# garymm/starflate

Measured on AMD Instinct MI355X. Metric: compress MiB/s + ratio vs zlib -6, 1 GiB synthetic; 1/2/4/8 GPU, higher is better.
Workload: dtype u8

## Files before the change

### starflate_amd/csrc/sf_capi.hip

```cpp
#include "../../include/starflate_hip.h"
#include "sf_device.h"

#include <dlfcn.h>
#include <stdio.h>
#include <stdlib.h>
#include <string.h>
#include <algorithm>
#include <memory>
#include <new>
#include <thread>
#include <vector>

struct sfh_ctx {
  int device = 0;
  hipStream_t stream = nullptr;
  sf::Workspace ws{};
  uint32_t cap_chunks = 0;
  uint32_t cap_batch = 0;
  uint32_t cap_dtok = 0;
  size_t seginfo_cap = 0;
  size_t sums_cap = 0;
  uint32_t last_chunks = 0;
  uint32_t last_block_bytes = 0;
  bool index_valid = false;
// ... 261 lines not shown
    SF_HIP(hipEventSynchronize(ctx->ev_batch[b % sfh_ctx::kPipe]), "wait for a batch");
    const size_t end = (size_t)ctx->h_tot[b % sfh_ctx::kPipe];
    if (end > pipe->cap) { pipe->overflow = true; return SFH_OK; }
    if (end > pipe->copied)
      SF_HIP(hipMemcpyAsync(pipe->dst + pipe->copied, (const uint8_t*)d_dst + pipe->copied, end - pipe->copied,
                            hipMemcpyDeviceToHost, ctx->s_out), "D2H");
    pipe->copied = end;
    return SFH_OK;
  };
  uint32_t bi = 0;
  for (uint32_t c0 = 0; c0 < nchunks; c0 += batch, ++bi) {
    const uint32_t nb = std::min(batch, nchunks - c0);
    const bool first = c0 == 0, last = c0 + nb == nchunks;
    const uint8_t* bsrc = (const uint8_t*)d_src + (size_t)c0 * sf::kChunk;
    const size_t bn = std::min((size_t)nb * sf::kChunk, n - (size_t)c0 * sf::kChunk);
    if (pipe && bn) {
      SF_HIP(hipMemcpyAsync(const_cast<uint8_t*>(bsrc), pipe->src + (size_t)c0 * sf::kChunk, bn, hipMemcpyHostToDevice, ctx->s_in), "H2D");
      SF_HIP(hipEventRecord(ctx->ev_in[bi % sfh_ctx::kPipe], ctx->s_in), "event");
      SF_HIP(hipStreamWaitEvent(s, ctx->ev_in[bi % sfh_ctx::kPipe], 0), "wait for the input");
    }
    sf::Workspace w = ctx->ws;
    w.offsets += c0;
    w.subidx += (size_t)c0 * 2 * sf::kSubRegions;
    sf::Options bo = ko;
    bo.final_stream = last ? ko.final_stream : 0u;
    hipEvent_t* ev = prof ? &ctx->ev[(size_t)bi * sfh_ctx::kEvPerBatch] : nullptr;
    if (ev) SF_HIP(hipEventRecord(ev[0], s), "event");
    SF_HIP(sf::launch_lz77(bsrc, bn, nb, w, bo, s), "launch k_lz77");
    if (ev) SF_HIP(hipEventRecord(ev[1], s), "event");
    SF_HIP(sf::launch_plan(bn, nb, w, bo, s), "launch k_plan");
    if (ev) SF_HIP(hipEventRecord(ev[2], s), "event");
    SF_HIP(sf::launch_scan(nb, w, sf::wrapper_header_bytes(o.container), !first, d_out_n, s), "launch k_scan");
    if (ev) SF_HIP(hipEventRecord(ev[3], s), "event");
    SF_HIP(sf::launch_emit(bsrc, bn, nb, w, (uint8_t*)d_dst, s), "launch k_emit");
    if (ev) SF_HIP(hipEventRecord(ev[4], s), "event");
    if (pipe) {
      if (bi >= 1 && (rc = drain(bi - 1)) != SFH_OK) return rc;
      SF_HIP(hipMemcpyAsync(&ctx->h_tot[bi % sfh_ctx::kPipe], d_out_n, sizeof(uint64_t), hipMemcpyDeviceToHost, s), "copy size");
      SF_HIP(hipEventRecord(ctx->ev_batch[bi % sfh_ctx::kPipe], s), "event");
    }
  }
  if (pipe && (rc = drain(bi - 1)) != SFH_OK) return rc;
  if (o.container) {
    SF_HIP(sf::launch_checksum((const uint8_t*)d_src, n, nchunks, o.container, ctx->ws.sums, s), "launch k_checksum");
    SF_HIP(sf::launch_wrap(ctx->ws.sums, nchunks, n, o.container, (uint8_t*)d_dst, d_out_n, nullptr, s), "launch k_wrap");
  }
  if (prof) {
    SF_HIP(hipEventRecord(ctx->ev[(size_t)nbatches * sfh_ctx::kEvPerBatch], s), "event");
    ctx->ev_batches = nbatches;
  }
  ctx->ev_valid = prof;
  ctx->index_valid = true;
  return mark_call_end(ctx, s);
}

int stage_tables(sfh_ctx* ctx, size_t bytes) {
  if (!ctx->ev_tab) SF_HIP(hipEventCreateWithFlags(&ctx->ev_tab, hipEventDisableTiming), "event");
  if (ctx->tab_pending) SF_HIP(hipEventSynchronize(ctx->ev_tab), "wait for the previous call's table copy");
  ctx->tab_pending = false;
  if (ctx->h_tab_cap < bytes) {
    if (ctx->h_tab) (void)hipHostFree(ctx->h_tab);
    ctx->h_tab = nullptr;
    ctx->h_tab_cap = 0;
    const hipError_t e = hipHostMalloc((void**)&ctx->h_tab, bytes, hipHostMallocDefault);
    if (e != hipSuccess) return fail(ctx, SFH_E_NOMEM, "pinned descriptor tables", e);
    ctx->h_tab_cap = bytes;
  }
// ... 123 lines not shown

  ctx->index_valid = false;
  ctx->last_chunks = lbs.back().nchunks;
  const bool prof = ctx->profiling != 0;
  if ((rc = order_behind_last_call(ctx, s)) != SFH_OK) return rc;
  SF_HIP(hipMemcpyAsync(ctx->d_tab, ctx->h_tab, bytes, hipMemcpyHostToDevice, s), "descriptor tables");
  SF_HIP(hipEventRecord(ctx->ev_tab, s), "event");
  ctx->tab_pending = true;
  const uint32_t nbatches = (uint32_t)lbs.size();
  ctx->ev_valid = false;
  if (prof) {
    const size_t need = (size_t)nbatches * sfh_ctx::kEvPerBatch + 1;
    while (ctx->ev.size() < need) {
      hipEvent_t e = nullptr;
      SF_HIP(hipEventCreate(&e), "event");
      ctx->ev.push_back(e);
    }
  }
  const uint64_t hdr = sf::wrapper_header_bytes(o.container);
  for (uint32_t bi = 0; bi < nbatches; ++bi) {
    const LaunchBatch& b = lbs[bi];
    const sf::BatchTables bt{d_strips + b.s0, b.nstrips, d_chunks + b.c0, d_items + b.i0, b.nitems};
    sf::Workspace w = ctx->ws;
    w.offsets += b.c0;
    w.subidx += (size_t)b.c0 * 2 * sf::kSubRegions;
    hipEvent_t* ev = prof ? &ctx->ev[(size_t)bi * sfh_ctx::kEvPerBatch] : nullptr;
    if (ev) SF_HIP(hipEventRecord(ev[0], s), "event");
    SF_HIP(sf::launch_lz77(nullptr, 0, b.nchunks, ctx->ws, ko, s, &bt), "launch k_lz77");
    if (ev) SF_HIP(hipEventRecord(ev[1], s), "event");
    SF_HIP(sf::launch_plan(0, b.nchunks, ctx->ws, ko, s, &bt), "launch k_plan");
    if (ev) SF_HIP(hipEventRecord(ev[2], s), "event");
    SF_HIP(sf::launch_scan(b.nchunks, w, hdr, false, d_out_n, s, &bt), "launch k_scan");
    if (ev) SF_HIP(hipEventRecord(ev[3], s), "event");
    SF_HIP(sf::launch_emit(nullptr, 0, b.nchunks, w, nullptr, s, &bt), "launch k_emit");
    if (ev) SF_HIP(hipEventRecord(ev[4], s), "event");
  }
  SF_HIP(sf::launch_batch_index(d_chunks, d_ixrows, d_items, ctx->ws.offsets, d_out_n, nchunks, ctx->d_bix, s), "launch k_batch_index");
  if (o.container) {
    SF_HIP(sf::launch_checksum_batch(d_chunks, nchunks, o.container, ctx->ws.sums, s), "launch k_checksum");
    SF_HIP(sf::launch_wrap_batch(ctx->ws.sums, d_wraps, (uint32_t)count, o.container, d_out_n, s), "launch k_wrap");
  }
  if (prof) {
    SF_HIP(hipEventRecord(ctx->ev[(size_t)nbatches * sfh_ctx::kEvPerBatch], s), "event");
    ctx->ev_batches = nbatches;
  }
  ctx->ev_valid = prof;
  ctx->bix_valid = true;
  ctx->bix_items = count;
  ctx->bix_entries = (size_t)nchunks + count;
  return mark_call_end(ctx, s);
}

int check_inflate_batch(sfh_ctx* ctx, size_t count, const void* const* srcs, const uint64_t* src_n, const uint64_t* index,
                        const uint32_t* subindex, void* const* dsts, const uint64_t* dst_n, const uint32_t* block_bytes,
                        uint32_t container, const uint32_t* status, bool dev) {
  if (!ctx || container > SFH_GZIP) return fail(ctx, SFH_E_INVALID_ARG, "argument (container)", hipSuccess);
  if (count == 0) return SFH_OK;
  if (!srcs || !src_n || !dsts || !dst_n || !status) return fail(ctx, SFH_E_INVALID_ARG, "null array", hipSuccess);
  if (count > ((size_t)1 << 31) - 1) return fail(ctx, SFH_E_INVALID_ARG, "too many items", hipSuccess);
  if (subindex && !index) return fail(ctx, SFH_E_INVALID_ARG, "a sub-index without an index", hipSuccess);
  if (dev && (((uintptr_t)index & 7) || ((uintptr_t)subindex & 3) || ((uintptr_t)status & 3)))
    return fail(ctx, SFH_E_INVALID_ARG, "device pointer alignment (index 8, sub-index 4, status 4)", hipSuccess);
  uint64_t segs = 0;
  for (size_t i = 0; i < count; ++i) {
    if ((!srcs[i] && src_n[i]) || (!dsts[i] && dst_n[i])) return fail(ctx, SFH_E_INVALID_ARG, "null item pointer", hipSuccess);
    if (dev && (((uintptr_t)srcs[i] & 3) || ((uintptr_t)dsts[i] & 15)))
      return fail(ctx, SFH_E_INVALID_ARG, "device pointer alignment (src 4, dst 16)", hipSuccess);
// ... 1005 lines not shown
```

### starflate_amd/csrc/sf_device.h

```cpp
#pragma once
#include <hip/hip_runtime.h>
#include <stdint.h>

namespace sf {

constexpr uint32_t kChunk = 32768;
constexpr uint32_t kWindow = 32768;
constexpr uint32_t kStep = 1024;
constexpr uint32_t kHashBits = 13;
constexpr uint32_t kMaxStrip = 1u << 24;
constexpr uint32_t kRegion = 512;
constexpr uint32_t kSubBytes = 1024;
constexpr uint32_t kCap = 16;
constexpr uint32_t kMinMatch = 4;
constexpr uint32_t kFar4 = 4096;
constexpr uint32_t kSkipSlack = 128;
constexpr uint32_t kSkipProbe = 2048;
constexpr uint32_t kItemsSkipped = 0x80000000u;
constexpr uint32_t kSubRegions = kChunk / kSubBytes;
constexpr uint32_t kTokMatch = 0x80000000u;
constexpr uint32_t kTokRegion = 0x40000000u;
constexpr uint32_t kItemTok = 0x8000u;
constexpr uint32_t kItemRegion = 0x4000u;
constexpr uint32_t kItemRegionShift = 9;
// ... 148 lines not shown
  uint32_t hist;
};
constexpr uint32_t kSegWrapped = 0x80000000u;
struct InflateStrip {
  uint32_t seg0, nseg;
};
struct InflateItem {
  const uint8_t* src;
  uint64_t src_n;
  uint64_t dst_n;
  uint64_t* implied;
  const uint64_t* ix0;
  uint32_t seg0, nseg;
  uint32_t wst;
  uint32_t want;
  uint32_t isize;
  uint32_t pad;
};
static_assert(sizeof(InflateSeg) == 48 && sizeof(InflateStrip) == 8 && sizeof(InflateItem) == 64, "decoder descriptor rows");
struct BatchTables {
  const BatchStrip* strips;
  uint32_t nstrips;
  const BatchChunk* chunks;
  BatchItem* items;
  uint32_t nitems;
};

hipError_t launch_lz77(const uint8_t* src, uint64_t n, uint32_t nchunks, const Workspace& ws,
                       const Options& opt, hipStream_t s, const BatchTables* bt = nullptr);
hipError_t launch_plan(uint64_t n, uint32_t nchunks, const Workspace& ws, const Options& opt,
                       hipStream_t s, const BatchTables* bt = nullptr);
hipError_t launch_scan(uint32_t nchunks, const Workspace& ws, uint64_t base, bool carry, uint64_t* d_total, hipStream_t s,
                       const BatchTables* bt = nullptr);
hipError_t launch_emit(const uint8_t* src, uint64_t n, uint32_t nchunks, const Workspace& ws,
                       uint8_t* dst, hipStream_t s, const BatchTables* bt = nullptr);
hipError_t launch_batch_index(const BatchChunk* chunks, const BatchIndexRow* rows, const BatchItem* pieces, const uint64_t* offsets,
                              const uint64_t* total, uint32_t nchunks, uint64_t* index, hipStream_t s);
hipError_t init_kernels();

uint32_t wrapper_header_bytes(uint32_t kind);
hipError_t launch_checksum(const uint8_t* src, uint64_t n, uint32_t nchunks, uint32_t kind, uint32_t* sums,
                           hipStream_t s);
hipError_t launch_wrap(const uint32_t* sums, uint32_t nchunks, uint64_t n, uint32_t kind, uint8_t* dst,
                       uint64_t* d_total, uint32_t* d_value, hipStream_t s);
hipError_t launch_checksum_batch(const BatchChunk* chunks, uint32_t nchunks, uint32_t kind, uint32_t* sums, hipStream_t s);
hipError_t launch_wrap_batch(const uint32_t* sums, const WrapItem* items, uint32_t nitems, uint32_t kind,
                             uint64_t* d_total, hipStream_t s);
hipError_t init_inflate_kernels();
hipError_t launch_inflate_tokens(const uint8_t* src, uint64_t src_n, const uint64_t* index, uint32_t nseg, uint64_t dst_n,
                                 uint32_t* tokens, SegInfo* info, uint32_t sps, bool speculate, hipStream_t s);
hipError_t launch_inflate_tokens_sub(const uint8_t* src, uint64_t src_n, const uint64_t* index, const uint32_t* subidx,
                                     uint32_t nseg, uint64_t dst_n, uint32_t* tokens, SegInfo* info, uint32_t sps,
                                     hipStream_t s);
hipError_t launch_inflate_bytes(const uint8_t* src, uint64_t src_n, uint32_t nseg, const uint32_t* tokens, SegInfo* info,
                                uint8_t* dst, uint32_t sps, hipStream_t s);
hipError_t launch_inflate_status(const SegInfo* info, uint32_t nseg, uint32_t* d_result, hipStream_t s);
hipError_t launch_inflate_tokens_batch(const InflateSeg* rows, uint32_t nseg, uint32_t* tokens, SegInfo* info, bool sub,
                                       bool speculate, hipStream_t s);
hipError_t launch_inflate_bytes_batch(const InflateSeg* rows, const InflateStrip* strips, uint32_t nstrips,
                                      const uint32_t* tokens, SegInfo* info, hipStream_t s);
hipError_t launch_inflate_head(InflateItem* items, uint32_t nitems, uint32_t container, InflateSeg* segs, BatchChunk* sums,
                               hipStream_t s);
hipError_t launch_inflate_fold(const InflateItem* items, uint32_t nitems, const SegInfo* info, const uint32_t* sums,
                               uint32_t container, uint32_t* status, hipStream_t s);

hipError_t run_lds_order_check(int op, uint32_t blocks, uint32_t iters, uint32_t* d_result, hipStream_t s);

// ... 5 lines not shown
```

### starflate_amd/csrc/sf_kernels.hip

```cpp
#include "sf_device.h"

#include <stdlib.h>

namespace sf {

__device__ __forceinline__ uint32_t len_symbol(uint32_t l3, uint32_t& ebits, uint32_t& eval) {
  if (l3 == 255) { ebits = 0; eval = 0; return 285; }
  if (l3 < 8) { ebits = 0; eval = 0; return 257 + l3; }
  const uint32_t e = (31 - __builtin_clz(l3)) - 2;
  ebits = e;
  eval = l3 & ((1u << e) - 1);
  return 257 + 4 * e + 4 + ((l3 >> e) & 3);
}
__device__ __forceinline__ uint32_t dist_symbol(uint32_t d1, uint32_t& ebits, uint32_t& eval) {
  if (d1 < 4) { ebits = 0; eval = 0; return d1; }
  const uint32_t hb = 31 - __builtin_clz(d1);
  const uint32_t e = hb - 1;
  ebits = e;
  eval = d1 & ((1u << e) - 1);
  return 2 * hb + ((d1 >> e) & 1);
}
__device__ __forceinline__ uint32_t dist_symbol_of(uint32_t d1) {
  const uint32_t x = d1 > 2u ? d1 : 2u;
  const uint32_t hb = 31 - __builtin_clz(x);
// ... 1314 lines not shown
      } else {
        q = (r - 1) / 6u;
        rem = (r - 1) - 6u * q;
        cnt = 1 + q + ((rem >= 3) ? 1u : rem);
      }
    }
    const uint32_t incl = wave_incl_add(cnt);
    uint32_t k = base + total + incl - cnt;
    auto put = [&](uint32_t sym, uint32_t ext) {
      S.rle_sym[k] = (uint8_t)sym;
      S.rle_ext[k] = (uint8_t)ext;
      atomicAdd(&S.clfreq[sym], 1u);
      ++k;
    };
    if (start) {
      if (v == 0) {
        for (uint32_t c = 0; c < q; ++c) put(18, 138 - 11);
        if (rem >= 11) put(18, rem - 11);
        else if (rem >= 3) put(17, rem - 3);
        else for (uint32_t c = 0; c < rem; ++c) put(0, 0);
      } else {
        put(v, 0);
        for (uint32_t c = 0; c < q; ++c) put(16, 6 - 3);
        if (rem >= 3) put(16, rem - 3);
        else for (uint32_t c = 0; c < rem; ++c) put(v, 0);
      }
    }
    total += (uint32_t)__builtin_amdgcn_readlane((int)incl, 63);
  }
  return total;
}

__constant__ uint8_t c_cl_order[19] = {16, 17, 18, 0, 8, 7, 9, 6, 10, 5, 11, 4, 12, 3, 13, 2, 14, 1, 15};

template <int MODE>
__device__ __forceinline__ void plan_chunk(uint64_t n_total, uint32_t nchunks,
                                           uint32_t* __restrict__ hist, const uint32_t* __restrict__ ntok,
                                           ChunkPlan* __restrict__ plan, ChunkCodes* __restrict__ codes,
                                           uint32_t strategy, uint32_t final_stream,
                                           uint64_t* __restrict__ stamps, PlanTree* __restrict__ ptree,
                                           const BatchChunk* __restrict__ bchunks) {
  __shared__ PlanSmem S;
  uint32_t* const s_header = S.key + kHeaderAt;
  uint64_t st_t = stamps ? __builtin_amdgcn_s_memtime() : 0;
  uint32_t st_k = 0;
  auto stamp = [&]() {
    if (stamps) {
      const uint64_t now = __builtin_amdgcn_s_memtime();
      if (threadIdx.x == 0 && st_k < 8) stamps[((uint64_t)nchunks + blockIdx.x) * 8 + st_k] = now - st_t;
      st_t = now;
      ++st_k;
    }
  };
  const uint32_t lane = threadIdx.x;
  const uint32_t chunk = blockIdx.x;
  uint32_t n_raw;
  bool fin;
  if (bchunks) {
    const BatchChunk B = bchunks[chunk];
    n_raw = B.n_raw;
    fin = (B.item & 1u) && final_stream;
  } else {
    const uint64_t cbase = (uint64_t)chunk * kChunk;
    n_raw = (uint32_t)((n_total - cbase) < (uint64_t)kChunk ? (n_total - cbase) : kChunk);
    fin = (chunk + 1 == nchunks) && final_stream;
  }

  PlanTree* const T = ptree + chunk;
  if constexpr (MODE == 2) {
    if (T->done) return;
  }
  if (MODE == 1 && strategy == 0 && n_raw != 0 && ntok[chunk] == 0) {
    ChunkCodes& C0 = codes[chunk];
    for (uint32_t s0 = lane; s0 < 320; s0 += 64) C0.lens[s0] = 0;
    if (lane == 0) {
      C0.header[0] = fin ? 1u : 0u;
      ChunkPlan P;
      P.btype = 0;
      P.out_bytes = n_raw + 5;
      P.header_bits = 3;
      P.body_bits = 0;
      plan[chunk] = P;
      T->done = 1;
    }
    return;
  }
  uint32_t rawf[4] = {0, 0, 0, 0};
  if constexpr (MODE == 1) {
#pragma unroll
    for (uint32_t q = 0; q < 4; ++q) rawf[q] = hist[(uint64_t)chunk * kHistStride + kHistLen + lane + 64 * q];
  }
  for (uint32_t s = lane; s < 320; s += 64) S.freq[s] = hist[(uint64_t)chunk * kHistStride + s];
  for (uint32_t s = lane; s < 320; s += 64) S.lens[s] = 0;
  __syncthreads();
  if constexpr (MODE == 1) {
#pragma unroll
    for (uint32_t q = 0; q < 4; ++q) {
      uint32_t eb, ev;
      if (rawf[q]) atomicAdd(&S.freq[len_symbol(lane + 64 * q, eb, ev)], rawf[q]);
    }
    __syncthreads();
    if (lane < 29) hist[(uint64_t)chunk * kHistStride + 257 + lane] = S.freq[257 + lane];
  }

  stamp();
  if (MODE == 1 && strategy == 0) {
    uint32_t fixb = 0, extra = 0, tot = 0;
    for (uint32_t s0 = lane; s0 < 286; s0 += 64) tot += S.freq[s0];
    tot = wave_sum(tot);
    const uint32_t ltot = est_log2(tot);
    uint32_t ent = 0;
    for (uint32_t s0 = lane; s0 < 286; s0 += 64) {
      const uint32_t f = S.freq[s0];
      if (f) ent += f * (ltot - est_log2(f));
      fixb += f * fixed_ll_len(s0);
      if (s0 >= 257) extra += f * len_extra_of_sym(s0 - 257);
    }
    const uint32_t g = lane < 30 ? S.freq[kHistD + lane] : 0u;
    const uint32_t nmat = wave_sum(g);
    if (g) ent += g * (est_log2(nmat) - est_log2(g));
    if (lane < 30) extra += g * dist_extra_of_sym(lane);
    const uint32_t extra_all = wave_sum(extra);
    const uint32_t est_bits = (wave_sum(ent) >> 8) + extra_all + kEstHeaderBits;
    const uint32_t fixbits = 3 + wave_sum(fixb) + extra_all + 5 * nmat;
    const uint32_t est_b = fin ? (est_bits + 7) / 8 : (est_bits + 3 + 7) / 8 + 4;
    const uint32_t fix_b = fin ? (fixbits + 7) / 8 : (fixbits + 3 + 7) / 8 + 4;
    const uint32_t sto_b = n_raw + 5;
    if (fix_b >= sto_b && est_b + kStoreMargin >= sto_b) {
      ChunkCodes& C0 = codes[chunk];
      for (uint32_t s0 = lane; s0 < 320; s0 += 64) C0.lens[s0] = 0;
      if (lane == 0) {
        C0.header[0] = fin ? 1u : 0u;
        ChunkPlan P;
        P.btype = 0;
        P.out_bytes = sto_b;
        P.header_bits = 3;
        P.body_bits = 0;
        plan[chunk] = P;
        T->done = 1;
      }
      return;
    }
  }
  if constexpr (MODE == 1) {
    const uint32_t m_ll = sort_symbols<5>(S, S.freq, 286, S.lens, lane);
    if (m_ll >= 2)
      for (uint32_t k = lane; k < m_ll; k += 64) {
        const uint32_t key = S.key[k];
        T->key_ll[k] = key;
        T->wt_ll[k] = (uint16_t)(key >> 9);
      }
    __syncthreads();
    const uint32_t m_d = sort_symbols<1>(S, S.freq + kHistD, 30, S.lens + 288, lane);
    if (m_d >= 2 && lane < m_d) {
      const uint32_t key = S.key[lane];
      T->key_d[lane] = key;
      T->wt_d[lane] = (uint16_t)(key >> 9);
    }
    if (lane == 0) { T->done = 0; T->m_ll = m_ll; T->m_d = m_d; }
    return;
// ... 66 lines not shown
    hclen = hclen < 4 ? 4u : hclen;
    if (lane == 0)
      or_bits(s_header, 0, (uint64_t)((fin ? 1u : 0u) | (2u << 1) | ((hlit - 257) << 3) | ((hdist - 1) << 8) | ((hclen - 4) << 13)));
    if (lane < hclen) or_bits(s_header, 17 + 3 * lane, (uint64_t)S.cl_lens[c_cl_order[lane]]);
    uint32_t bitbase = 17 + 3 * hclen;
#pragma unroll
    for (uint32_t g = 0; g < 5; ++g) {
      if (g * 64 >= nitems) break;
      const uint32_t k = g * 64 + lane;
      uint32_t nb = 0;
      uint64_t v = 0;
      if (k < nitems) {
        const uint32_t sy = S.rle_sym[k];
        const uint32_t c = S.cl_code[sy];
        const uint32_t cl = c >> 16;
        const uint32_t eb = sy == 16 ? 2u : sy == 17 ? 3u : sy == 18 ? 7u : 0u;
        v = (uint64_t)(c & 0xFFFF) | ((uint64_t)S.rle_ext[k] << cl);
        nb = cl + eb;
      }
      const uint32_t incl = wave_incl_add(nb);
      if (nb) or_bits(s_header, bitbase + incl - nb, v);
      bitbase += (uint32_t)__builtin_amdgcn_readlane((int)incl, 63);
    }
    if (lane == 0) S.cnt[0] = bitbase;
  }
  __syncthreads();

  stamp();
  const uint32_t dyn_hbits = S.cnt[0];
  const uint32_t dyn_bits = dyn_hbits + dyn_body;
  const uint32_t fix_bits = 3 + fix_body;
  const uint32_t dyn_bytes = fin ? (dyn_bits + 7) / 8 : (dyn_bits + 3 + 7) / 8 + 4;
  const uint32_t fix_bytes = fin ? (fix_bits + 7) / 8 : (fix_bits + 3 + 7) / 8 + 4;
  const uint32_t sto_bytes = n_raw + 5;
  uint32_t bt;
  if (strategy == 1) bt = 0;
  else if (strategy == 2) bt = 1;
  else if (strategy == 3) bt = 2;
  else {
    bt = 0;
    uint32_t best = sto_bytes;
    if (fix_bytes < best) { bt = 1; best = fix_bytes; }
    if (dyn_bytes < best) { bt = 2; best = dyn_bytes; }
  }

  ChunkCodes& C = codes[chunk];
  for (uint32_t s = lane; s < 320; s += 64) C.lens[s] = S.lens[s];
  __syncthreads();
  if (bt == 1) {
    for (uint32_t s = lane; s < 320; s += 64) S.lens[s] = s < 288 ? (uint8_t)fixed_ll_len(s) : (uint8_t)5;
    if (lane == 0) s_header[0] = (fin ? 1u : 0u) | (1u << 1);
    __syncthreads();
  } else if (bt == 0) {
    if (lane == 0) s_header[0] = fin ? 1u : 0u;
    __syncthreads();
  }
  canonical_codes(S.lens, 288, C.lcode, lane);
  canonical_codes(S.lens + 288, 32, C.dcode, lane);
  const uint32_t hbits = bt == 2 ? dyn_hbits : 3;
  for (uint32_t k = lane; k < (hbits + 31) / 32; k += 64) C.header[k] = s_header[k];
  if (lane == 0) {
    ChunkPlan P;
    P.btype = bt;
    P.out_bytes = bt == 0 ? sto_bytes : bt == 1 ? fix_bytes : dyn_bytes;
    P.header_bits = hbits;
    P.body_bits = bt == 1 ? fix_body : dyn_body;
    plan[chunk] = P;
// ... 77 lines not shown
  __syncthreads();
  if (wave == 0) {
    const uint32_t x = lane < K3_TILES ? s_tile[lane] : 0u;
    const uint32_t r = wave_incl_add(x);
    if (lane < K3_TILES) s_tile[lane] = r - x;
    if (lane == K3_TILES - 1) s_tile[K3_TILES] = r;
  }
  __syncthreads();
#pragma unroll
  for (uint32_t k = 0; k < K3_TILES; ++k) {
    const uint32_t c = k * K3_THREADS + t;
    if (c < nchunks) offsets[c] = base + s_tile[k] + s_wt[k][wave] + ex[k];
  }
  if (t == 0) {
    const uint64_t all = base + s_tile[K3_TILES];
    if constexpr (!BATCH) *total = all;
    offsets[nchunks] = all;
  }
  if constexpr (BATCH) {
    __syncthreads();
    for (uint32_t i = t; i < nitems; i += K3_THREADS) {
      BatchItem& I = bitems[i];
      const uint64_t g0 = offsets[I.chunk0], g1 = offsets[I.chunk0 + I.nchunks];
      const uint64_t start = I.carry ? total[I.out] : hdr;
      I.shift = start - g0;
      total[I.out] = start + (g1 - g0);
    }
  }
}

constexpr uint32_t K4_THREADS = 512;
constexpr uint32_t K4_WAVES = K4_THREADS / 64;
constexpr uint32_t K4_IPT = 8;
constexpr uint32_t K4_STAGE_WORDS = 9392;
static_assert(4 * K4_STAGE_WORDS >= kChunk + kChunk / 8 + 640 + 16 + 8, "k_emit: stage holds the largest chunk");
static_assert(4 * (4 * K4_STAGE_WORDS + 4 * (288 + 32 + 256 + 2 * 8 + kSubRegions) + 512) <= 160 * 1024, "k_emit: four workgroups per CU");

__device__ __forceinline__ void literal_bits(uint32_t byte, const uint32_t* lcode, uint64_t& value, uint32_t& nb) {
  const uint32_t lc = lcode[byte];
  value = lc & 0xFFFF;
  nb = lc >> 16;
}
__device__ __forceinline__ uint32_t lenlut_entry(uint32_t l3, const uint32_t* lcode) {
  uint32_t le, lv;
  const uint32_t lc = lcode[len_symbol(l3, le, lv)];
  const uint32_t p = lc >> 16;
  return (lc & 0xFFFFu) | (lv << p) | ((p + le) << 24);
}
__device__ __forceinline__ void match_bits(uint32_t l3, uint32_t d1, const uint32_t* lenlut, const uint32_t* dcode,
                                           uint64_t& value, uint32_t& nb) {
  uint32_t de, dv;
  const uint32_t ds = dist_symbol(d1, de, dv);
  const uint32_t le = lenlut[l3], dc = dcode[ds];
  uint32_t p = le >> 24;
  uint64_t v = le & 0xFFFFFFu;
  v |= (uint64_t)(dc & 0xFFFF) << p;
  p += dc >> 16;
  v |= (uint64_t)dv << p;
  p += de;
  value = v;
  nb = p;
}

template <bool BATCH>
__global__ __launch_bounds__(K4_THREADS, 4) void k_emit(const uint8_t* __restrict__ src, uint64_t n_total,
                                                     uint32_t , uint16_t* items,
                                                     const uint32_t* __restrict__ nitems_in,
                                                     const uint32_t* __restrict__ ntok_in,
                                                     const ChunkPlan* __restrict__ plan,
                                                     const ChunkCodes* __restrict__ codes,
                                                     const uint64_t* __restrict__ offsets,
                                                     const uint32_t* __restrict__ rtok,
                                                     uint32_t* __restrict__ subidx,
                                                     uint8_t* __restrict__ dst_all,
                                                     const BatchChunk* __restrict__ bchunks,
                                                     const BatchItem* __restrict__ bitems) {
  __shared__ __attribute__((aligned(16))) uint32_t s_stage[K4_STAGE_WORDS];
  __shared__ uint32_t s_lcode[288];
  __shared__ uint32_t s_dcode[32];
  __shared__ uint32_t s_tab[1024];
  __shared__ uint32_t s_wtot[2][K4_WAVES];
  __shared__ uint32_t s_rtok[kSubRegions];
  static_assert(K4_THREADS == 512, "one table entry per thread and kind");
  constexpr uint32_t kTabLit = 512, kTabLen = 768, kTabDistN = 510;

  const uint32_t t = threadIdx.x, lane = t & 63;
  const uint32_t wave = (uint32_t)__builtin_amdgcn_readfirstlane((int)(t >> 6));
  const uint32_t chunk = blockIdx.x;
  const ChunkPlan P = plan[chunk];
  const uint8_t* csrc;
  uint8_t* dst;
  uint64_t off = offsets[chunk];
  uint32_t n_raw;
  if constexpr (BATCH) {
    const BatchChunk B = bchunks[chunk];
    const BatchItem& I = bitems[B.item >> 1];
    csrc = B.src;
    n_raw = B.n_raw;
    dst = I.dst;
    off += I.shift;
  } else {
    const uint64_t cbase = (uint64_t)chunk * kChunk;
    csrc = src + cbase;
    n_raw = (uint32_t)((n_total - cbase) < (uint64_t)kChunk ? (n_total - cbase) : kChunk);
    dst = dst_all;
  }
  const ChunkCodes& C = codes[chunk];
  uint32_t pre_code = t < 288 ? C.lcode[t] : (t < 320 ? C.dcode[t - 288] : 0u);
  uint32_t pre_rtok = t < kSubRegions ? rtok[(uint64_t)chunk * kSubRegions + t] : 0u;
  const uint32_t pre_ntok = ntok_in[chunk], pre_nit = nitems_in[chunk];
  asm volatile("" : "+v"(pre_code), "+v"(pre_rtok));

  uint32_t* const sub = subidx + (uint64_t)chunk * 2 * kSubRegions;
  if (P.btype == 0) {
    if (t < 2 * kSubRegions) sub[t] = 0;
// ... 33 lines not shown
        d4[k] = r;
      }
      const uint32_t done16 = head16 + 16 * nvec;
      if (t < n_raw - done16) d[done16 + t] = sp[done16 + t];
      return;
    }
    const uint32_t head = (uint32_t)((4 - ((uintptr_t)d & 3)) & 3);
    const uint32_t h = head < n_raw ? head : n_raw;
    if (t < h) d[t] = sp[t];
    const uint32_t nd = (n_raw - h) / 4;
    uint32_t* d32 = reinterpret_cast<uint32_t*>(d + h);
    const uint32_t* s32 = reinterpret_cast<const uint32_t*>(sp);
    const uint32_t full_src_words = n_raw / 4;
    for (uint32_t k = t; k < nd; k += K4_THREADS) {
      const uint32_t ob = h + 4 * k;
      const uint32_t w = ob >> 2;
      uint32_t lo = s32[w], hi = 0;
      if ((ob & 3) != 0) {
        if (w + 1 < full_src_words) hi = s32[w + 1];
        else
          for (uint32_t b = 0; b < 4 && 4 * (w + 1) + b < n_raw; ++b) hi |= (uint32_t)sp[4 * (w + 1) + b] << (8 * b);
      }
      d32[k] = __builtin_amdgcn_alignbyte(hi, lo, ob & 3);
    }
    const uint32_t done = h + 4 * nd;
    if (t < n_raw - done) d[done + t] = sp[done + t];
    return;
  }

  const uint32_t sh = (uint32_t)(off & 3);
  const uint32_t nwords = (sh + P.out_bytes + 3) / 4;
  {
    uint4* z = reinterpret_cast<uint4*>(s_stage);
    for (uint32_t k = t; k < (nwords + 2 + 3) / 4 && k < K4_STAGE_WORDS / 4; k += K4_THREADS) z[k] = make_uint4(0, 0, 0, 0);
  }
  if (t < 288) s_lcode[t] = pre_code;
  else if (t < 320) s_dcode[t - 288] = pre_code;
  if (t < kSubRegions) {
    s_rtok[t] = pre_rtok;
    sub[2 * t + 1] = pre_rtok;
  }
  __syncthreads();
  if (t < 256) {
    const uint32_t le = lenlut_entry(t, s_lcode);
    s_tab[kTabLen + t] = (le & 0xFFFFFu) | ((le >> 24) << 20);
    s_tab[kTabLit + t] = (pre_code & 0xFFFFu) | ((pre_code >> 16) << 20);
  }
  if (t < kTabDistN) {
    const uint32_t sym = dist_symbol_of(t < 256 ? t : (t - 254) << 7);
    const uint32_t dc = s_dcode[sym];
    s_tab[t] = (dc & 0xFFFFu) | ((dc >> 16) << 20) | (dist_extra_of_sym(sym) << 25);
  } else {
    s_tab[t] = 0;
  }
  {
    uint8_t* sb = reinterpret_cast<uint8_t*>(s_stage) + sh;
    const uint8_t* hb = reinterpret_cast<const uint8_t*>(C.header);
    const uint32_t hbytes = (P.header_bits + 7) / 8;
    for (uint32_t k = t; k < hbytes; k += K4_THREADS) sb[k] = hb[k];
  }
  __syncthreads();

  const uint32_t ntok = pre_ntok;
  const uint32_t nit = pre_nit & ~kItemsSkipped;
  const uint16_t* it = items + (uint64_t)chunk * kChunk;
  if (pre_nit & kItemsSkipped) {
    uint16_t* const wr = items + (uint64_t)chunk * kChunk;
    for (uint32_t pos = t; pos < nit; pos += K4_THREADS) {
      const uint32_t b = csrc[pos];
      wr[pos] = (uint16_t)(kItemTok | ((pos & (kSubBytes - 1)) == 0 ? (b | kItemRegion | ((pos / kSubBytes) << kItemRegionShift)) : b));
    }
    __threadfence_block();
    __syncthreads();
  }
  uint32_t running = 8 * sh + P.header_bits;
  uint32_t buf = 0;
  uint4 q_next = make_uint4(0, 0, 0, 0);
  if (nit) q_next = *reinterpret_cast<const uint4*>(it + t * K4_IPT);
  for (uint32_t b0 = 0; b0 < nit; b0 += K4_THREADS * K4_IPT, buf ^= 1) {
    const uint32_t i0 = b0 + t * K4_IPT;
    const uint4 q = q_next;
    const bool full = b0 + K4_THREADS * K4_IPT <= nit;
    if (b0 + K4_THREADS * K4_IPT < nit) q_next = *reinterpret_cast<const uint4*>(it + i0 + K4_THREADS * K4_IPT);
    const uint32_t e[K4_IPT] = {q.x & 0xFFFFu, q.x >> 16, q.y & 0xFFFFu, q.y >> 16, q.z & 0xFFFFu, q.z >> 16, q.w & 0xFFFFu, q.w >> 16};
    uint32_t val[K4_IPT], nb[K4_IPT], mine = 0;
    uint32_t ent[K4_IPT];
#pragma unroll
    for (uint32_t k = 0; k < K4_IPT; ++k) {
      const uint32_t cur = e[k];
      static_assert(kItemHead == 0x100 && kTabLen == kTabLit + 0x100 && kTabLit == 0x200, "a token's low nine bits are its table index");
      uint32_t itok = (cur & 0x1FFu) | kTabLit, idist = min(cur, 254u + (cur >> 7));
      asm volatile("" : "+v"(itok), "+v"(idist));
      ent[k] = s_tab[cur >= kItemTok ? itok : idist];
    }
    asm volatile("" : "+v"(ent[0]), "+v"(ent[1]), "+v"(ent[2]), "+v"(ent[3]), "+v"(ent[4]), "+v"(ent[5]), "+v"(ent[6]), "+v"(ent[7]));
    auto both = [](uint32_t w) { return w & (w << 1) & 0x80008000u; };
    uint32_t flagged = both(q.x) | both(q.y) | both(q.z) | both(q.w);
    if (!full) {
      uint32_t left = nit - i0;
      left = i0 < nit ? left : 0u;
#pragma unroll
      for (uint32_t k = 0; k < K4_IPT; ++k) ent[k] = k < left ? ent[k] : 0u;
      flagged = 1;
    }
#pragma unroll
    for (uint32_t k = 0; k < K4_IPT; ++k) {
      const uint32_t en = ent[k];
      const uint32_t dl = __builtin_amdgcn_ubfe(en, 20, 5), de = en >> 25;
      val[k] = (__builtin_amdgcn_ubfe(e[k], 0, de) << dl) | (en & 0xFFFFFu);
      nb[k] = dl + de;
      mine += nb[k];
    }
    uint32_t starts = 0;
    if (flagged) {
      uint32_t i_now = i0;
      asm volatile("" : "+v"(i_now));
#pragma unroll
      for (uint32_t k = 0; k < K4_IPT; ++k)
        starts |= ((e[k] & (kItemTok | kItemRegion)) == (kItemTok | kItemRegion) && i_now + k < nit) ? 1u << k : 0u;
    }
    const uint32_t incl = wave_incl_add(mine);
    if (lane == 63) s_wtot[buf][wave] = incl;
    __syncthreads();
    uint32_t pre = 0, all = 0;
#pragma unroll
    for (uint32_t w = 0; w < K4_WAVES; ++w) {
      const uint32_t v = s_wtot[buf][w];
      if (w < wave) pre += v;
      all += v;
    }
    const uint32_t pos = running + pre + incl - mine;
    if (starts) {
      uint32_t pk = pos;
#pragma unroll
      for (uint32_t k = 0; k < K4_IPT; ++k) {
        if ((starts >> k) & 1) sub[2 * ((e[k] >> kItemRegionShift) & 31u)] = pk - 8 * sh;
        pk += nb[k];
      }
    }
    uint32_t wi = pos >> 5, ab = pos & 31;
    uint64_t acc = 0;
    auto put = [&](uint32_t v32, uint32_t n) {
      acc |= (uint64_t)v32 << ab;
      ab += n;
      if (ab >= 32) {
        atomicOr(&s_stage[wi++], (uint32_t)acc);
        acc >>= 32;
        ab -= 32;
      }
    };
#pragma unroll
    for (uint32_t k = 0; k < K4_IPT; ++k) put(val[k], nb[k]);
    if (ab) atomicOr(&s_stage[wi], (uint32_t)acc);
    running += all;
  }
  __syncthreads();
  if (t < kSubRegions && s_rtok[t] >= ntok) sub[2 * t] = running - 8 * sh;
  if (t == 0) {
    const uint32_t eob = s_lcode[256];
    or_bits(s_stage, running, eob & 0xFFFF);
    const uint32_t endbit = running + (eob >> 16);
    if (!(C.header[0] & 1u)) {
      const uint32_t byte = (endbit + 3 + 7) / 8;
      or_bits(s_stage, 8 * (byte + 2), 0xFFFFull);
    }
  }
  __syncthreads();

  uint8_t* gbase = dst + (off - sh);
  uint32_t* g32 = reinterpret_cast<uint32_t*>(gbase);
  const uint32_t lo_b = sh, hi_b = sh + P.out_bytes;
// ... 51 lines not shown
  hipLaunchKernelGGL(k_plan_sort, dim3(nchunks), dim3(64), 0, s, n, nchunks, ws.hist, ws.ntok, ws.plan, ws.codes,
                     opt.strategy, opt.final_stream, (uint64_t*)nullptr, ws.ptree, bchunks);
  hipLaunchKernelGGL(k_plan_merge, dim3((nchunks + 63) / 64), dim3(64), 0, s, nchunks, ws.ptree);
  hipLaunchKernelGGL(k_plan_finish, dim3(nchunks), dim3(64), 0, s, n, nchunks, ws.hist, ws.ntok, ws.plan, ws.codes,
                     opt.strategy, opt.final_stream, ws.stamps, ws.ptree, bchunks);
  return hipGetLastError();
}
hipError_t launch_scan(uint32_t nchunks, const Workspace& ws, uint64_t base, bool carry, uint64_t* d_total, hipStream_t s,
                       const BatchTables* bt) {
  if (nchunks > kBatchChunks) return hipErrorInvalidValue;
  if (bt)
    hipLaunchKernelGGL(k_scan<true>, dim3(1), dim3(K3_THREADS), 0, s, nchunks, ws.plan, base, 0u, ws.offsets, d_total, bt->items,
                       bt->nitems);
  else
    hipLaunchKernelGGL(k_scan<false>, dim3(1), dim3(K3_THREADS), 0, s, nchunks, ws.plan, base, carry ? 1u : 0u, ws.offsets, d_total,
                       (BatchItem*)nullptr, 0u);
  return hipGetLastError();
}
__global__ __launch_bounds__(256) void k_batch_index(const BatchChunk* __restrict__ chunks, const BatchIndexRow* __restrict__ rows,
                                                     const BatchItem* __restrict__ pieces, const uint64_t* __restrict__ offsets,
                                                     const uint64_t* __restrict__ total, uint32_t nchunks, uint64_t* __restrict__ index) {
  const uint32_t c = blockIdx.x * 256 + threadIdx.x;
  if (c >= nchunks) return;
  const BatchIndexRow R = rows[c];
  const uint64_t e = (uint64_t)c + R.item;
  index[e] = offsets[c] + pieces[R.piece].shift;
  if (chunks[c].item & 1u) index[e + 1] = total[R.item];
}
hipError_t launch_batch_index(const BatchChunk* chunks, const BatchIndexRow* rows, const BatchItem* pieces, const uint64_t* offsets,
                              const uint64_t* total, uint32_t nchunks, uint64_t* index, hipStream_t s) {
  hipLaunchKernelGGL(k_batch_index, dim3((nchunks + 255) / 256), dim3(256), 0, s, chunks, rows, pieces, offsets, total, nchunks, index);
  return hipGetLastError();
}
hipError_t launch_emit(const uint8_t* src, uint64_t n, uint32_t nchunks, const Workspace& ws,
                       uint8_t* dst, hipStream_t s, const BatchTables* bt) {
  if (bt)
    hipLaunchKernelGGL(k_emit<true>, dim3(nchunks), dim3(K4_THREADS), 0, s, src, n, nchunks, ws.items, ws.nitems, ws.ntok,
                       ws.plan, ws.codes, ws.offsets, ws.rtok, ws.subidx, dst, bt->chunks, (const BatchItem*)bt->items);
  else
    hipLaunchKernelGGL(k_emit<false>, dim3(nchunks), dim3(K4_THREADS), 0, s, src, n, nchunks, ws.items, ws.nitems, ws.ntok,
                       ws.plan, ws.codes, ws.offsets, ws.rtok, ws.subidx, dst, (const BatchChunk*)nullptr,
                       (const BatchItem*)nullptr);
  return hipGetLastError();
}

}
```

Baseline: 218,500.

## Shrink k_emit LDS stage under auto strategy and vectorize token table lookup

Templates k_emit on its LDS stage size. Under the default strategy the stage drops to a smaller size that still covers a stored-block fallback, which allows more waves per SIMD. The table-index computation now runs on packed 16-bit pairs, and each table entry carries the total bit count so the per-item extra-bit width needs no add. Region-start bookkeeping uses a bitmask with a fast path for a single start per thread and only rescans items when several starts occur. The cost is more code paths and a dependence on the plan never exceeding the small stage outside the forced strategies.

```diff
diff --git a/starflate_amd/csrc/sf_capi.hip b/starflate_amd/csrc/sf_capi.hip
--- a/starflate_amd/csrc/sf_capi.hip
+++ b/starflate_amd/csrc/sf_capi.hip
@@ -317,7 +317,7 @@
     if (ev) SF_HIP(hipEventRecord(ev[2], s), "event");
     SF_HIP(sf::launch_scan(nb, w, sf::wrapper_header_bytes(o.container), !first, d_out_n, s), "launch k_scan");
     if (ev) SF_HIP(hipEventRecord(ev[3], s), "event");
-    SF_HIP(sf::launch_emit(bsrc, bn, nb, w, (uint8_t*)d_dst, s), "launch k_emit");
+    SF_HIP(sf::launch_emit(bsrc, bn, nb, w, bo, (uint8_t*)d_dst, s), "launch k_emit");
     if (ev) SF_HIP(hipEventRecord(ev[4], s), "event");
     if (pipe) {
       if (bi >= 1 && (rc = drain(bi - 1)) != SFH_OK) return rc;
@@ -507,7 +507,7 @@
     if (ev) SF_HIP(hipEventRecord(ev[2], s), "event");
     SF_HIP(sf::launch_scan(b.nchunks, w, hdr, false, d_out_n, s, &bt), "launch k_scan");
     if (ev) SF_HIP(hipEventRecord(ev[3], s), "event");
-    SF_HIP(sf::launch_emit(nullptr, 0, b.nchunks, w, nullptr, s, &bt), "launch k_emit");
+    SF_HIP(sf::launch_emit(nullptr, 0, b.nchunks, w, ko, nullptr, s, &bt), "launch k_emit");
     if (ev) SF_HIP(hipEventRecord(ev[4], s), "event");
   }
   SF_HIP(sf::launch_batch_index(d_chunks, d_ixrows, d_items, ctx->ws.offsets, d_out_n, nchunks, ctx->d_bix, s), "launch k_batch_index");
diff --git a/starflate_amd/csrc/sf_device.h b/starflate_amd/csrc/sf_device.h
--- a/starflate_amd/csrc/sf_device.h
+++ b/starflate_amd/csrc/sf_device.h
@@ -204,7 +204,7 @@
                        hipStream_t s, const BatchTables* bt = nullptr);
 hipError_t launch_scan(uint32_t nchunks, const Workspace& ws, uint64_t base, bool carry, uint64_t* d_total, hipStream_t s,
                        const BatchTables* bt = nullptr);
-hipError_t launch_emit(const uint8_t* src, uint64_t n, uint32_t nchunks, const Workspace& ws,
+hipError_t launch_emit(const uint8_t* src, uint64_t n, uint32_t nchunks, const Workspace& ws, const Options& opt,
                        uint8_t* dst, hipStream_t s, const BatchTables* bt = nullptr);
 hipError_t launch_batch_index(const BatchChunk* chunks, const BatchIndexRow* rows, const BatchItem* pieces, const uint64_t* offsets,
                               const uint64_t* total, uint32_t nchunks, uint64_t* index, hipStream_t s);
diff --git a/starflate_amd/csrc/sf_kernels.hip b/starflate_amd/csrc/sf_kernels.hip
--- a/starflate_amd/csrc/sf_kernels.hip
+++ b/starflate_amd/csrc/sf_kernels.hip
@@ -1370,6 +1370,7 @@
 }
 
 __constant__ uint8_t c_cl_order[19] = {16, 17, 18, 0, 8, 7, 9, 6, 10, 5, 11, 4, 12, 3, 13, 2, 14, 1, 15};
+constexpr uint32_t kStoredExtra = 5;
 
 template <int MODE>
 __device__ __forceinline__ void plan_chunk(uint64_t n_total, uint32_t nchunks,
@@ -1415,7 +1416,7 @@
       C0.header[0] = fin ? 1u : 0u;
       ChunkPlan P;
       P.btype = 0;
-      P.out_bytes = n_raw + 5;
+      P.out_bytes = n_raw + kStoredExtra;
       P.header_bits = 3;
       P.body_bits = 0;
       plan[chunk] = P;
@@ -1463,7 +1464,7 @@
     const uint32_t fixbits = 3 + wave_sum(fixb) + extra_all + 5 * nmat;
     const uint32_t est_b = fin ? (est_bits + 7) / 8 : (est_bits + 3 + 7) / 8 + 4;
     const uint32_t fix_b = fin ? (fixbits + 7) / 8 : (fixbits + 3 + 7) / 8 + 4;
-    const uint32_t sto_b = n_raw + 5;
+    const uint32_t sto_b = n_raw + kStoredExtra;
     if (fix_b >= sto_b && est_b + kStoreMargin >= sto_b) {
       ChunkCodes& C0 = codes[chunk];
       for (uint32_t s0 = lane; s0 < 320; s0 += 64) C0.lens[s0] = 0;
@@ -1596,7 +1597,7 @@
   const uint32_t fix_bits = 3 + fix_body;
   const uint32_t dyn_bytes = fin ? (dyn_bits + 7) / 8 : (dyn_bits + 3 + 7) / 8 + 4;
   const uint32_t fix_bytes = fin ? (fix_bits + 7) / 8 : (fix_bits + 3 + 7) / 8 + 4;
-  const uint32_t sto_bytes = n_raw + 5;
+  const uint32_t sto_bytes = n_raw + kStoredExtra;
   uint32_t bt;
   if (strategy == 1) bt = 0;
   else if (strategy == 2) bt = 1;
@@ -1740,9 +1741,28 @@
 constexpr uint32_t K4_THREADS = 512;
 constexpr uint32_t K4_WAVES = K4_THREADS / 64;
 constexpr uint32_t K4_IPT = 8;
-constexpr uint32_t K4_STAGE_WORDS = 9392;
-static_assert(4 * K4_STAGE_WORDS >= kChunk + kChunk / 8 + 640 + 16 + 8, "k_emit: stage holds the largest chunk");
-static_assert(4 * (4 * K4_STAGE_WORDS + 4 * (288 + 32 + 256 + 2 * 8 + kSubRegions) + 512) <= 160 * 1024, "k_emit: four workgroups per CU");
+constexpr uint32_t K4_STAGE_FORCED = 9392;
+constexpr uint32_t K4_STAGE_AUTO = 8200;
+static_assert(4 * K4_STAGE_FORCED >= 3 + kChunk + kChunk / 8 + 640 + 16 + 8, "k_emit: the stage holds the largest chunk");
+static_assert(4 * K4_STAGE_AUTO >= 3 + kChunk + kStoredExtra - 1 + 16 + 8, "k_emit: the small stage holds the largest chunk "
+              "plan_chunk codes under strategy 0");
+static_assert(K4_STAGE_FORCED % 4 == 0 && K4_STAGE_AUTO % 4 == 0, "the stage is zeroed in 16-byte steps");
+template <uint32_t STAGE_WORDS>
+struct EmitLds {
+  alignas(16) uint32_t stage[STAGE_WORDS];
+  uint32_t lcode[288];
+  uint32_t dcode[32];
+  uint32_t tab[1024];
+  uint32_t wtot[2][K4_WAVES];
+  uint32_t rtok[kSubRegions];
+};
+template <uint32_t STAGE_WORDS>
+constexpr uint32_t k4_waves_per_simd() { return STAGE_WORDS == K4_STAGE_AUTO ? 8 : 6; }
+static_assert(k4_waves_per_simd<K4_STAGE_AUTO>() / 2 * sizeof(EmitLds<K4_STAGE_AUTO>) <= 160 * 1024, "k_emit: four workgroups per CU");
+static_assert(k4_waves_per_simd<K4_STAGE_FORCED>() / 2 * sizeof(EmitLds<K4_STAGE_FORCED>) <= 160 * 1024, "k_emit: three workgroups per CU");
+
+typedef uint16_t u16x2 __attribute__((ext_vector_type(2)));
+typedef int16_t s16x2 __attribute__((ext_vector_type(2)));
 
 __device__ __forceinline__ void literal_bits(uint32_t byte, const uint32_t* lcode, uint64_t& value, uint32_t& nb) {
   const uint32_t lc = lcode[byte];
@@ -1770,8 +1790,8 @@
   nb = p;
 }
 
-template <bool BATCH>
-__global__ __launch_bounds__(K4_THREADS, 4) void k_emit(const uint8_t* __restrict__ src, uint64_t n_total,
+template <bool BATCH, uint32_t STAGE_WORDS>
+__global__ __launch_bounds__(K4_THREADS, k4_waves_per_simd<STAGE_WORDS>()) void k_emit(const uint8_t* __restrict__ src, uint64_t n_total,
                                                      uint32_t , uint16_t* items,
                                                      const uint32_t* __restrict__ nitems_in,
                                                      const uint32_t* __restrict__ ntok_in,
@@ -1783,12 +1803,13 @@
                                                      uint8_t* __restrict__ dst_all,
                                                      const BatchChunk* __restrict__ bchunks,
                                                      const BatchItem* __restrict__ bitems) {
-  __shared__ __attribute__((aligned(16))) uint32_t s_stage[K4_STAGE_WORDS];
-  __shared__ uint32_t s_lcode[288];
-  __shared__ uint32_t s_dcode[32];
-  __shared__ uint32_t s_tab[1024];
-  __shared__ uint32_t s_wtot[2][K4_WAVES];
-  __shared__ uint32_t s_rtok[kSubRegions];
+  __shared__ EmitLds<STAGE_WORDS> L;
+  uint32_t(&s_stage)[STAGE_WORDS] = L.stage;
+  uint32_t(&s_lcode)[288] = L.lcode;
+  uint32_t(&s_dcode)[32] = L.dcode;
+  uint32_t(&s_tab)[1024] = L.tab;
+  uint32_t(&s_wtot)[2][K4_WAVES] = L.wtot;
+  uint32_t(&s_rtok)[kSubRegions] = L.rtok;
   static_assert(K4_THREADS == 512, "one table entry per thread and kind");
   constexpr uint32_t kTabLit = 512, kTabLen = 768, kTabDistN = 510;
 
@@ -1888,7 +1909,7 @@
   const uint32_t nwords = (sh + P.out_bytes + 3) / 4;
   {
     uint4* z = reinterpret_cast<uint4*>(s_stage);
-    for (uint32_t k = t; k < (nwords + 2 + 3) / 4 && k < K4_STAGE_WORDS / 4; k += K4_THREADS) z[k] = make_uint4(0, 0, 0, 0);
+    for (uint32_t k = t; k < (nwords + 2 + 3) / 4 && k < STAGE_WORDS / 4; k += K4_THREADS) z[k] = make_uint4(0, 0, 0, 0);
   }
   if (t < 288) s_lcode[t] = pre_code;
   else if (t < 320) s_dcode[t - 288] = pre_code;
@@ -1899,13 +1920,13 @@
   __syncthreads();
   if (t < 256) {
     const uint32_t le = lenlut_entry(t, s_lcode);
-    s_tab[kTabLen + t] = (le & 0xFFFFFu) | ((le >> 24) << 20);
-    s_tab[kTabLit + t] = (pre_code & 0xFFFFu) | ((pre_code >> 16) << 20);
+    s_tab[kTabLen + t] = (le & 0xFFFFFu) | (le >> 24) * (1u << 20 | 1u << 27);
+    s_tab[kTabLit + t] = (pre_code & 0xFFFFu) | (pre_code >> 16) * (1u << 20 | 1u << 27);
   }
   if (t < kTabDistN) {
     const uint32_t sym = dist_symbol_of(t < 256 ? t : (t - 254) << 7);
     const uint32_t dc = s_dcode[sym];
-    s_tab[t] = (dc & 0xFFFFu) | ((dc >> 16) << 20) | (dist_extra_of_sym(sym) << 25);
+    s_tab[t] = (dc & 0xFFFFu) | ((dc >> 16) << 20) | (((dc >> 16) + dist_extra_of_sym(sym)) << 27);
   } else {
     s_tab[t] = 0;
   }
@@ -1938,42 +1959,54 @@
     const uint4 q = q_next;
     const bool full = b0 + K4_THREADS * K4_IPT <= nit;
     if (b0 + K4_THREADS * K4_IPT < nit) q_next = *reinterpret_cast<const uint4*>(it + i0 + K4_THREADS * K4_IPT);
-    const uint32_t e[K4_IPT] = {q.x & 0xFFFFu, q.x >> 16, q.y & 0xFFFFu, q.y >> 16, q.z & 0xFFFFu, q.z >> 16, q.w & 0xFFFFu, q.w >> 16};
+    const uint32_t qd[K4_IPT / 2] = {q.x, q.y, q.z, q.w};
     uint32_t val[K4_IPT], nb[K4_IPT], mine = 0;
     uint32_t ent[K4_IPT];
 #pragma unroll
-    for (uint32_t k = 0; k < K4_IPT; ++k) {
-      const uint32_t cur = e[k];
+    for (uint32_t j = 0; j < K4_IPT / 2; ++j) {
       static_assert(kItemHead == 0x100 && kTabLen == kTabLit + 0x100 && kTabLit == 0x200, "a token's low nine bits are its table index");
-      uint32_t itok = (cur & 0x1FFu) | kTabLit, idist = min(cur, 254u + (cur >> 7));
-      asm volatile("" : "+v"(itok), "+v"(idist));
-      ent[k] = s_tab[cur >= kItemTok ? itok : idist];
+      static_assert(kItemTok == 0x8000, "bit 15 tells a token's first item from a distance");
+      const u16x2 w = __builtin_bit_cast(u16x2, qd[j]);
+      const uint32_t itok = (qd[j] & 0x01FF01FFu) | (kTabLit * 0x10001u);
+      const u16x2 idist = __builtin_elementwise_min(w, (u16x2)(w >> (uint16_t)7) + (uint16_t)254);
+      uint32_t tok = __builtin_bit_cast(uint32_t, __builtin_bit_cast(s16x2, w) >> (int16_t)15);
+      asm volatile("" : "+v"(tok));
+      const uint32_t idx = (tok & itok) | (~tok & __builtin_bit_cast(uint32_t, idist));
+      const uint32_t by = __builtin_bit_cast(uint32_t, (u16x2)(__builtin_bit_cast(u16x2, idx) << (uint16_t)2));
+      ent[2 * j] = *reinterpret_cast<const uint32_t*>(reinterpret_cast<const uint8_t*>(s_tab) + (by & 0xFFFFu));
+      ent[2 * j + 1] = *reinterpret_cast<const uint32_t*>(reinterpret_cast<const uint8_t*>(s_tab) + (by >> 16));
     }
     asm volatile("" : "+v"(ent[0]), "+v"(ent[1]), "+v"(ent[2]), "+v"(ent[3]), "+v"(ent[4]), "+v"(ent[5]), "+v"(ent[6]), "+v"(ent[7]));
     auto both = [](uint32_t w) { return w & (w << 1) & 0x80008000u; };
-    uint32_t flagged = both(q.x) | both(q.y) | both(q.z) | both(q.w);
+    auto sbit = [](uint32_t k) { return (k & 1) ? 15 + k : k; };
+    uint32_t starts = (both(q.x) >> 15) | (both(q.y) >> 13) | (both(q.z) >> 11) | (both(q.w) >> 9);
     if (!full) {
       uint32_t left = nit - i0;
       left = i0 < nit ? left : 0u;
 #pragma unroll
-      for (uint32_t k = 0; k < K4_IPT; ++k) ent[k] = k < left ? ent[k] : 0u;
-      flagged = 1;
-    }
+      for (uint32_t k = 0; k < K4_IPT; ++k) {
+        ent[k] = k < left ? ent[k] : 0u;
+        starts &= k < left ? ~0u : ~(1u << sbit(k));
+      }
+    }
+    const uint32_t s0 = starts ? (uint32_t)__builtin_ctz(starts) : 32u;
+    const bool walk = __ballot((starts & (starts - 1)) != 0) != 0;
+    uint32_t off0 = 0;
 #pragma unroll
     for (uint32_t k = 0; k < K4_IPT; ++k) {
       const uint32_t en = ent[k];
-      const uint32_t dl = __builtin_amdgcn_ubfe(en, 20, 5), de = en >> 25;
-      val[k] = (__builtin_amdgcn_ubfe(e[k], 0, de) << dl) | (en & 0xFFFFFu);
-      nb[k] = dl + de;
+      const uint32_t dl = en >> 20, n = en >> 27;
+      val[k] = (__builtin_amdgcn_ubfe(qd[k / 2], 16 * (k & 1), (n - dl) & 31u) << (dl & 31u)) | (en & 0xFFFFFu);
+      nb[k] = n;
+      asm volatile("" : "+v"(val[k]), "+v"(nb[k]));
+      off0 = s0 == sbit(k) ? mine : off0;
       mine += nb[k];
     }
-    uint32_t starts = 0;
-    if (flagged) {
-      uint32_t i_now = i0;
-      asm volatile("" : "+v"(i_now));
-#pragma unroll
-      for (uint32_t k = 0; k < K4_IPT; ++k)
-        starts |= ((e[k] & (kItemTok | kItemRegion)) == (kItemTok | kItemRegion) && i_now + k < nit) ? 1u << k : 0u;
+    uint32_t region0;
+    {
+      const uint32_t j = (s0 >> 1) & 3u;
+      const uint32_t w = j == 0 ? q.x : j == 1 ? q.y : j == 2 ? q.z : q.w;
+      region0 = (w >> ((s0 & 16u) + kItemRegionShift)) & 31u;
     }
     const uint32_t incl = wave_incl_add(mine);
     if (lane == 63) s_wtot[buf][wave] = incl;
@@ -1986,13 +2019,19 @@
       all += v;
     }
     const uint32_t pos = running + pre + incl - mine;
-    if (starts) {
+    if (walk) {
+      const uint4 r = *reinterpret_cast<const uint4*>(it + i0);
+      const uint32_t rd[K4_IPT / 2] = {r.x, r.y, r.z, r.w};
       uint32_t pk = pos;
 #pragma unroll
       for (uint32_t k = 0; k < K4_IPT; ++k) {
-        if ((starts >> k) & 1) sub[2 * ((e[k] >> kItemRegionShift) & 31u)] = pk - 8 * sh;
+        const uint32_t e = (rd[k / 2] >> (16 * (k & 1))) & 0xFFFFu;
+        if ((e & (kItemTok | kItemRegion)) == (kItemTok | kItemRegion) && i0 + k < nit)
+          sub[2 * ((e >> kItemRegionShift) & 31u)] = pk - 8 * sh;
         pk += nb[k];
       }
+    } else if (starts) {
+      sub[2 * region0] = pos + off0 - 8 * sh;
     }
     uint32_t wi = pos >> 5, ab = pos & 31;
     uint64_t acc = 0;
@@ -2110,15 +2149,16 @@
   hipLaunchKernelGGL(k_batch_index, dim3((nchunks + 255) / 256), dim3(256), 0, s, chunks, rows, pieces, offsets, total, nchunks, index);
   return hipGetLastError();
 }
-hipError_t launch_emit(const uint8_t* src, uint64_t n, uint32_t nchunks, const Workspace& ws,
+hipError_t launch_emit(const uint8_t* src, uint64_t n, uint32_t nchunks, const Workspace& ws, const Options& opt,
                        uint8_t* dst, hipStream_t s, const BatchTables* bt) {
-  if (bt)
-    hipLaunchKernelGGL(k_emit<true>, dim3(nchunks), dim3(K4_THREADS), 0, s, src, n, nchunks, ws.items, ws.nitems, ws.ntok,
-                       ws.plan, ws.codes, ws.offsets, ws.rtok, ws.subidx, dst, bt->chunks, (const BatchItem*)bt->items);
-  else
-    hipLaunchKernelGGL(k_emit<false>, dim3(nchunks), dim3(K4_THREADS), 0, s, src, n, nchunks, ws.items, ws.nitems, ws.ntok,
-                       ws.plan, ws.codes, ws.offsets, ws.rtok, ws.subidx, dst, (const BatchChunk*)nullptr,
-                       (const BatchItem*)nullptr);
+  const auto launch = [&](auto kernel) {
+    hipLaunchKernelGGL(kernel, dim3(nchunks), dim3(K4_THREADS), 0, s, src, n, nchunks, ws.items, ws.nitems, ws.ntok, ws.plan,
+                       ws.codes, ws.offsets, ws.rtok, ws.subidx, dst, bt ? bt->chunks : (const BatchChunk*)nullptr,
+                       bt ? (const BatchItem*)bt->items : (const BatchItem*)nullptr);
+  };
+  const bool forced = opt.strategy == 2 || opt.strategy == 3;
+  if (bt) forced ? launch(k_emit<true, K4_STAGE_FORCED>) : launch(k_emit<true, K4_STAGE_AUTO>);
+  else forced ? launch(k_emit<false, K4_STAGE_FORCED>) : launch(k_emit<false, K4_STAGE_AUTO>);
   return hipGetLastError();
 }
 
```

New measurement: 224,300 (median of 6 runs). 2.7% higher.
